# jlogan03/interpn

Hardware: AMD Instinct MI355X
Metric: Mpoints/sec (f64) per GPU + achieved HBM GB/s vs roofline, 3D linear-regular (higher is better)
Workload: dtype f64

## Files before the change

interpn_amd/csrc/abi_layout.hip:

```cpp
#include "abi_internal.h"

using namespace interpn;
using namespace interpn_abi;

namespace interpn_abi {

static bool grid_is_l1_resident(const GridDesc& g) {
  return g.nvals * (g.dtype == kF64 ? 8u : 4u) <= 16u * 1024u;
}

int maybe_build_cubic_tiles(interpn_hip_interp* h) {
  GridDesc& g = h->desc;
  const char* env = getenv("INTERPN_HIP_BRICKS");
  if (env && !strcmp(env, "off")) return INTERPN_HIP_OK;
  if (!(env && strlen(env) == 2) && grid_is_l1_resident(g)) return INTERPN_HIP_OK;
  static const int cand[5][2] = {{4, 4}, {2, 4}, {2, 2}, {1, 4}, {1, 1}};
  size_t free_b = 0, total_b = 0;
  if (hipMemGetInfo(&free_b, &total_b) != hipSuccess) free_b = (size_t)8 << 30;
  int best = -1;
  double best_cost = 0;
  for (int c = 0; c < 5; ++c) {
    const int si = cand[c][0], sj = cand[c][1];
    if (env && strlen(env) == 2 && !(env[0] - '0' == si && env[1] - '0' == sj)) continue;
    unsigned nb[2];
// ... 154 lines not shown
    } else if (fits(bone)) {
      if (bone <= l2_sized || b22 > l2_sized) { si = 1; sj = 1; j4 = f32; }
      else if (b12 <= l2_sized) { si = 1; sj = 2; }
      else { si = 2; sj = 2; }
    } else if (fits(b12)) { si = 1; sj = 2; }
    else if (fits(b22)) { si = 2; sj = 2; }
    else return INTERPN_HIP_OK;
  }
  size_t bytes;
  if (j4) {
    bytes = bj4;
    for (int k = 0; k < 3; ++k) g.brick_nb[k] = nbj4[k];
    g.brick_nb[3] = 0;
    si = sj = 1;
  } else if (cell) {
    bytes = bcell;
    for (int k = 0; k < 4; ++k) g.brick_nb[k] = nbc[k];
    si = sj = 1;
  } else {
    brick_geometry(g, si, sj, g.brick_nb, &bytes);
    g.brick_nb[3] = 0;
  }
  if (bytes / esz >= 0xFFFFFFFFull) return INTERPN_HIP_OK;
  if (bytes > free_b / 2) return INTERPN_HIP_OK;
  g.brick_step[0] = si;
  g.brick_step[1] = sj;
  g.brick_cell = j4 ? 2 : (cell ? 1 : 0);
  hipError_t e = pool_alloc(h->device, &h->bricks_owned, bytes);
  if (e != hipSuccess) { (void)hipGetLastError(); h->bricks_owned = nullptr; g.brick_cell = 0; return INTERPN_HIP_OK; }
  HIP_TRY(build_bricks(g, h->bricks_owned, nullptr));
  HIP_TRY(hipStreamSynchronize(nullptr));
  g.bricks = h->bricks_owned;
  g.sweep_bricks = nullptr;
  int wi = 0, wj = 0, wcell = 0;
  if (!(env && !strcmp(env, "off")) && sweep_layout(g, &wi, &wj, &wcell)) {
    unsigned nbs[3];
    size_t bsw = 0;
    if (wcell == 2) brick_j4_geometry(g, nbs, &bsw);
    else brick_geometry(g, wi, wj, nbs, &bsw);
    if (g.brick_cell == wcell && g.brick_step[0] == wi && g.brick_step[1] == wj) {
      g.sweep_bricks = g.bricks;
    } else if (bsw / esz < 0xFFFFFFFFull && bsw <= free_b / 4 && pool_alloc(h->device, &h->sweep_owned, bsw) == hipSuccess) {
      GridDesc t = g;
      t.brick_cell = wcell;
      t.brick_step[0] = wi;
      t.brick_step[1] = wj;
      for (int k = 0; k < 3; ++k) t.brick_nb[k] = nbs[k];
      t.brick_nb[3] = 0;
      if (build_bricks(t, h->sweep_owned, nullptr) == hipSuccess && hipStreamSynchronize(nullptr) == hipSuccess) {
        g.sweep_bricks = h->sweep_owned;
      } else {
        (void)hipGetLastError();
        pool_free(h->device, h->sweep_owned);
        h->sweep_owned = nullptr;
      }
    } else {
      (void)hipGetLastError();
      h->sweep_owned = nullptr;
    }
    if (g.sweep_bricks) {
      g.sweep_step[0] = wi;
      g.sweep_step[1] = wj;
      g.sweep_cell = wcell;
      for (int k = 0; k < 3; ++k) g.sweep_nb[k] = nbs[k];
      g.sweep_table_bytes = bsw;
    }
  }
  return INTERPN_HIP_OK;
}

}
```

interpn_amd/csrc/abi_options.hip:

```cpp
#include "abi_internal.h"

using namespace interpn;
using namespace interpn_abi;

namespace interpn_abi {

bool option_access(LaunchConfig& c, const char* name, long long* value, bool set) {
  struct Opt { const char* name; int* field; long long lo, hi; };
  const Opt opts[] = {
      {"blocks_per_cu", &c.blocks_per_cu, 1, 65536},
      {"iters_per_block", &c.iters_per_block, 0, 65536},
      {"ppl", &c.ppl, 0, 2},
      {"axis_regs", &c.axis_regs, -1, 2},
      {"force_generic", &c.force_generic, 0, 1},
      {"generic_runtime", &c.generic_runtime, 0, 1},
      {"generic_vec", &c.generic_vec, -1, 1},
      {"persistent", &c.persistent, 0, 1},
      {"axis_lds_kb", &c.axis_lds_kb, -1, 60},
      {"binned", &c.binned, -1, 1},
      {"deal", &c.deal, 0, 1},
      {"bin_slice_log2", &c.bin_slice_log2, 16, 27},
      {"column", &c.column, -1, 1},
      {"column_part", &c.column_part, 0, 1 << 20},
      {"column_threads", &c.column_threads, 256, 1024},
// ... 150 lines not shown
    for (const auto& sl : hm->bin_slots) {
      const unsigned char* base = static_cast<const unsigned char*>(sl.scratch);
      if (!sl.busy && word && base && word >= base && word + sizeof(unsigned) <= base + sl.bytes) idle = true;
    }
    *value = -1;
    if (idle) {
      DeviceGuard guard(h->device);
      if (!guard.ok()) return INTERPN_HIP_ERR_NO_DEVICE;
      unsigned w = 0;
      if (hipDeviceSynchronize() != hipSuccess || hipMemcpy(&w, word, sizeof(w), hipMemcpyDeviceToHost) != hipSuccess) { (void)hipGetLastError(); return INTERPN_HIP_ERR_INVALID_ARGUMENT; }
      *value = w ? 1 : 0;
    }
    return INTERPN_HIP_OK;
  }
  if (!strcmp(name, "sweep_probe_streak")) {
    interpn_hip_interp* hm = const_cast<interpn_hip_interp*>(h);
    std::lock_guard<std::mutex> lk(hm->bin_mu);
    *value = hm->sampling.streak;
    return INTERPN_HIP_OK;
  }
  if (!strcmp(name, "sweep_cell")) { *value = h->desc.sweep_bricks ? h->desc.sweep_cell : 0; return INTERPN_HIP_OK; }
  if (!strcmp(name, "dev_pci")) {
    int dom = 0, bus = 0, dv = 0;
    if (hipDeviceGetAttribute(&dom, hipDeviceAttributePciDomainID, h->device) != hipSuccess ||
        hipDeviceGetAttribute(&bus, hipDeviceAttributePciBusId, h->device) != hipSuccess ||
        hipDeviceGetAttribute(&dv, hipDeviceAttributePciDeviceId, h->device) != hipSuccess) {
      (void)hipGetLastError();
      *value = -1;
    } else {
      *value = ((long long)dom << 16) | ((long long)(bus & 0xFF) << 8) | (long long)(dv & 0xFF);
    }
    return INTERPN_HIP_OK;
  }
  if (!strcmp(name, "sweep_layout")) { *value = h->desc.sweep_bricks ? h->desc.sweep_step[0] * 10 + h->desc.sweep_step[1] : 0; return INTERPN_HIP_OK; }
  if (!strcmp(name, "scratch_allocs")) { *value = h->scratch_allocs.load(); return INTERPN_HIP_OK; }
  if (!strcmp(name, "scratch_bytes")) {
    interpn_hip_interp* hm = const_cast<interpn_hip_interp*>(h);
    std::lock_guard<std::mutex> lk(hm->bin_mu);
    long long tot = 0;
    for (const auto& sl : hm->bin_slots) tot += (long long)sl.bytes;
    *value = tot;
    return INTERPN_HIP_OK;
  }
  LaunchConfig c = h->desc.cfg;
  return option_access(c, name, value, false) ? INTERPN_HIP_OK : INTERPN_HIP_ERR_INVALID_ARGUMENT;
}

int interpn_hip_kernel_name(const interpn_hip_interp* h, char* buf, size_t buflen) {
  if (!h || !buf || buflen == 0) return INTERPN_HIP_ERR_INVALID_ARGUMENT;
  const KernelTag t = h->desc.tag;
  if (!t.name) {
    buf[0] = 0;
    return INTERPN_HIP_OK;
  }
  std::string out = std::string("interpn::") + t.name + "<" + (h->desc.dtype == kF64 ? "double" : "float");
  for (int k = 0; k < t.nargs; ++k) {
    out += ", ";
    if (t.bool_mask & (1u << k)) out += t.args[k] ? "true" : "false";
    else out += std::to_string(t.args[k]);
  }
  out += ">";
  snprintf(buf, buflen, "%s", out.c_str());
  return INTERPN_HIP_OK;
}

size_t interpn_hip_table_bytes(const interpn_hip_interp* h, int* step_i, int* step_j) {
// ... 23 lines not shown
```

interpn_amd/csrc/interpn_device.h:

```cpp
#pragma once

#include <hip/hip_runtime.h>
#include <stdint.h>

#include "cubic_cell_record.h"

namespace interpn {

constexpr int kMaxDims = 8;
constexpr unsigned long long kNoBadIndex = ~0ull;

enum Sat : int { kSatNone = 0, kSatLow = 1, kSatHigh = 2 };

__device__ __forceinline__ void wave_sync() {
  __builtin_amdgcn_fence(__ATOMIC_ACQ_REL, "wavefront");
  __builtin_amdgcn_wave_barrier();
  __builtin_amdgcn_fence(__ATOMIC_ACQ_REL, "wavefront");
}

template <typename V>
__device__ __forceinline__ V stream_load(const V* p) { return __builtin_nontemporal_load(p); }
template <typename V>
__device__ __forceinline__ void stream_store(V* p, V v) { __builtin_nontemporal_store(v, p); }

// ... 40 lines not shown
__device__ __forceinline__ Leaf<T, W> load_leaf(const T* __restrict__ p) {
  typedef typename LeafVec<T, W>::type V;
  V x = *reinterpret_cast<const V*>(p);
  Leaf<T, W> r;
#pragma unroll
  for (int i = 0; i < W; ++i) r.v[i] = x[i];
  return r;
}

template <typename T>
__device__ __forceinline__ bool regular_floc(T x, T start, T step, T* floc_out) {
  T floc = dev_floor<T>((x - start) / step);
  *floc_out = floc;
  return (floc >= (T)-9223372036854775808.0) && (floc < (T)9223372036854775808.0);
}

template <typename T>
__device__ __forceinline__ int clamp_loc(T floc_shifted, int dimmax) {
  const T big = sizeof(T) == 8 ? (T)2147483647.0 : (T)2147483520.0;
  T c = floc_shifted;
  c = c > (T)0 ? c : (T)0;
  c = c < big ? c : big;
  int li = (int)c;
  return li < dimmax ? li : dimmax;
}

template <typename T>
struct StepCell {
  T t;
  int loc;
  bool exact;
};

__device__ __forceinline__ bool exponent_within_256(double a) {
  const unsigned e = ((unsigned)__double2hiint(a) >> 20) & 0x7FFu;
  return e - (1023u - 256u) < 512u;
}

template <bool FMA>
__device__ __forceinline__ StepCell<double> step_cell_fast(double x, double start, double step, double rstep, int dimmax) {
  StepCell<double> r;
  const double qt = (x - start) * rstep;
  const double d = __builtin_amdgcn_fract(qt);
  r.exact = (__builtin_fabs(d - 0.5) < 0.5 - 0x1p-20) && (__builtin_fabs(qt) < 0x1p31);
  int li = (int)qt;
  li = li > 0 ? li : 0;
  li = li < dimmax ? li : dimmax;
  r.loc = li;
  const double lf = (double)li;
  const double izl = mul_add<FMA>(step, lf, start);
  const double a = x - izl;
  r.exact = r.exact && exponent_within_256(a);
  const double q0 = a * rstep;
  const double r0 = __builtin_fma(-step, q0, a);
  const double q1 = __builtin_fma(r0, rstep, q0);
  const double r1 = __builtin_fma(-step, q1, a);
  r.t = __builtin_fma(r1, rstep, q1);
  return r;
}

template <typename T>
struct StepCellIndex {
  T a;
  int loc;
  bool exact;
};
template <bool FMA>
__device__ __forceinline__ StepCellIndex<double> step_cell_index(double x, double start, double step, double rstep, int dimmax) {
  StepCellIndex<double> r;
  const double qt = (x - start) * rstep;
  const double d = __builtin_amdgcn_fract(qt);
  r.exact = (__builtin_fabs(d - 0.5) < 0.5 - 0x1p-20) && (__builtin_fabs(qt) < 0x1p31);
  int li = (int)qt;
  li = li > 0 ? li : 0;
  li = li < dimmax ? li : dimmax;
  r.loc = li;
  const double izl = mul_add<FMA>(step, (double)li, start);
  r.a = x - izl;
  r.exact = r.exact && exponent_within_256(r.a);
  return r;
}
__device__ __forceinline__ double step_cell_quotient(double a, double step, double rstep) {
  const double q0 = a * rstep;
  const double r0 = __builtin_fma(-step, q0, a);
  const double q1 = __builtin_fma(r0, rstep, q0);
  const double r1 = __builtin_fma(-step, q1, a);
  return __builtin_fma(r1, rstep, q1);
}

__device__ __forceinline__ bool exponent_within_24(float a) {
  const unsigned e = (__float_as_uint(a) >> 23) & 0xFFu;
  return e - (127u - 24u) < 48u;
}

template <bool FMA>
__device__ __forceinline__ StepCell<float> step_cell_fast(float x, float start, float step, float rstep, int dimmax) {
  StepCell<float> r;
  const float qt = (x - start) * rstep;
  const float d = __builtin_amdgcn_fractf(qt);
  const float margin = __builtin_fmaf(__builtin_fabsf(qt), 0x1p-21f, 0x1p-21f);
  r.exact = __builtin_fabsf(d - 0.5f) + margin < 0.5f;
  int li = (int)qt;
  li = li > 0 ? li : 0;
  li = li < dimmax ? li : dimmax;
  r.loc = li;
  const float lf = (float)li;
  const float izl = mul_add<FMA>(step, lf, start);
  const float a = x - izl;
  r.exact = r.exact && exponent_within_24(a);
  const float q0 = a * rstep;
  const float r0 = __builtin_fmaf(-step, q0, a);
  const float q1 = __builtin_fmaf(r0, rstep, q0);
  const float r1 = __builtin_fmaf(-step, q1, a);
  r.t = __builtin_fmaf(r1, rstep, q1);
  return r;
}

template <bool FMA>
__device__ __forceinline__ StepCellIndex<float> step_cell_index(float x, float start, float step, float rstep, int dimmax) {
  StepCellIndex<float> r;
  const float qt = (x - start) * rstep;
  const float d = __builtin_amdgcn_fractf(qt);
  const float margin = __builtin_fmaf(__builtin_fabsf(qt), 0x1p-21f, 0x1p-21f);
  r.exact = __builtin_fabsf(d - 0.5f) + margin < 0.5f;
  int li = (int)qt;
  li = li > 0 ? li : 0;
  li = li < dimmax ? li : dimmax;
  r.loc = li;
  const float izl = mul_add<FMA>(step, (float)li, start);
  r.a = x - izl;
  r.exact = r.exact && exponent_within_24(r.a);
  return r;
}
__device__ __forceinline__ float step_cell_quotient(float a, float step, float rstep) {
  const float q0 = a * rstep;
  const float r0 = __builtin_fmaf(-step, q0, a);
  const float q1 = __builtin_fmaf(r0, rstep, q0);
  const float r1 = __builtin_fmaf(-step, q1, a);
  return __builtin_fmaf(r1, rstep, q1);
}

__device__ __forceinline__ bool floor_quotient_fast(double a0, double rb, double* floc) {
  const double qt = a0 * rb;
  const double d = __builtin_amdgcn_fract(qt);
  *floc = __builtin_floor(qt);
  return (__builtin_fabs(d - 0.5) < 0.5 - 0x1p-20) && (__builtin_fabs(qt) < 0x1p31);
}
__device__ __forceinline__ bool floor_quotient_fast(float a0, float rb, float* floc) {
  const float qt = a0 * rb;
  const float d = __builtin_amdgcn_fractf(qt);
  *floc = __builtin_floorf(qt);
  return __builtin_fabsf(d - 0.5f) + __builtin_fmaf(__builtin_fabsf(qt), 0x1p-21f, 0x1p-21f) < 0.5f;
}
__device__ __forceinline__ bool divide_fast(double a, double b, double rb, double* q) {
  const double q0 = a * rb;
  const double r0 = __builtin_fma(-b, q0, a);
  const double q1 = __builtin_fma(r0, rb, q0);
  const double r1 = __builtin_fma(-b, q1, a);
  *q = __builtin_fma(r1, rb, q1);
  return exponent_within_256(a);
}
__device__ __forceinline__ bool divide_fast(float a, float b, float rb, float* q) {
  const float q0 = a * rb;
  const float r0 = __builtin_fmaf(-b, q0, a);
  const float q1 = __builtin_fmaf(r0, rb, q0);
  const float r1 = __builtin_fmaf(-b, q1, a);
// ... 449 lines not shown
```

interpn_amd/csrc/interpn_host.h:

```cpp
#pragma once

#include <hip/hip_runtime.h>
#include <stddef.h>

#include <initializer_list>

namespace interpn {

enum Method : int { kLinear = 0, kCubic = 1, kNearest = 2 };
enum OneDimMethod : int { kLinear1D = 16, kLinearHoldLast1D = 17, kLeft1D = 18, kRight1D = 19, kNearest1D = 20 };
inline bool is_one_dim(int method) { return method >= kLinear1D && method <= kNearest1D; }
enum Kind : int { kRegular = 0, kRectilinear = 1 };
enum DType : int { kF64 = 0, kF32 = 1 };

struct LaunchConfig {
  int num_cus = 256;
  int num_xcds = 8;
  long long l2_bytes = 4ll << 20;
  long long lds_per_cu = 160ll << 10;
  long long lds_per_wg = 64ll << 10;
  int blocks_per_cu = 8;
  int iters_per_block = 0;
  int ppl = 0;
  int axis_regs = -1;
// ... 61 lines not shown
  int n[8] = {0};
  double start[8] = {0};
  double step[8] = {0};
  const void* vals = nullptr;
  size_t nvals = 0;
  const void* grid[8] = {nullptr};
  size_t grid_total = 0;
  const void* axis_image = nullptr;
  unsigned axis_image_bytes = 0;
  unsigned axis_alloc_bytes = 0;
  unsigned axis_g_off[8] = {0};
  unsigned axis_tab_off[8] = {0};
  int axis_buckets[8] = {0};
  double axis_g0[8] = {0};
  double axis_scale[8] = {0};
  unsigned axis_ltab_off[8] = {0};
  double axis_lscale[8] = {0};
  int axis_lscan[8] = {0};
  unsigned axis_rec_off[8] = {0};
  unsigned axis_rec_base = 0;
  unsigned axis_rec_bytes = 0;
  int axis_rec_compact = 0;
  unsigned axis_recg_off[8] = {0};
  unsigned axis_crec_off[8] = {0};
  unsigned axis_crec_bytes = 0;
  const void* bricks = nullptr;
  int rec1_buckets = 0;
  double rec1_scale = 0.0;
  int brick_step[2] = {2, 2};
  unsigned brick_nb[4] = {0, 0, 0, 0};
  const void* bricks11 = nullptr;
  unsigned bricks11_nb[2] = {0, 0};
  int brick_cell = 0;
  const void* sweep_bricks = nullptr;
  int sweep_step[2] = {0, 0};
  int sweep_cell = 0;
  unsigned sweep_nb[3] = {0, 0, 0};
  size_t sweep_table_bytes = 0;
  double bound_lo[8] = {0};
  double bound_hi[8] = {0};
  int unrep_status = 7;
  double od_start = 0, od_step = 0, od_stop = 0, od_rstep = 0;
  int od_fast = 0;
  int od_M = 0;
  double od_g0 = 0, od_scale = 0;
  size_t od_g_off = 0, od_tab_off = 0, od_table_bytes = 0;
  LaunchConfig cfg;
  mutable KernelTag tag;
  mutable int last_lattice_path = -1;
  mutable int last_points_path = -1;
  mutable int last_binned = 0;
};

inline unsigned brick_iters(const GridDesc& g, size_t npts, int points_per_lane, int setup) {
  unsigned iters = g.cfg.iters_per_block > 0 ? (unsigned)g.cfg.iters_per_block : (setup == 2 ? 8u : (setup == 1 ? 4u : 1u));
  const size_t rows = (npts + (size_t)256 * points_per_lane - 1) / ((size_t)256 * points_per_lane);
  while ((rows + iters - 1) / iters > (1u << 23)) iters *= 2;
  return iters;
}

constexpr unsigned long long kNoBadIndexHost = ~0ull;

constexpr size_t kMaxGridLdsBytes = 20 * 1024;
constexpr size_t kMaxGridLdsBytesWide = 60 * 1024;

struct Thresholds {
  size_t table_l2_sized;
  size_t table_l2_share;
  double table_l2_model;
  size_t binned_table_min;
  size_t binned_points_min;
// ... 188 lines not shown
```

interpn_amd/csrc/k_linear_brick.hip:

```cpp
#include <cstdlib>

#include "linear_brick.h"

namespace interpn {

static unsigned bricks_along(int n, int step) {
  if (step == 1) return (unsigned)(n - 1);
  if (step == 2) return (unsigned)((n - 1) / 2 + 1);
  return (unsigned)((n - 2) / step + 1);
}

void brick_geometry(const GridDesc& g, int si, int sj, unsigned nb[3], size_t* bytes) {
  const int N = g.ndims;
  const int kw = g.dtype == kF64 ? 4 : 8;
  nb[0] = bricks_along(g.n[N - 3], si);
  nb[1] = bricks_along(g.n[N - 2], sj);
  nb[2] = bricks_along(g.n[N - 1], kw - 1);
  size_t lead = 1;
  for (int d = 0; d < N - 3; ++d) lead *= (size_t)g.n[d];
  *bytes = lead * nb[0] * nb[1] * nb[2] * 128;
}

void brick_cell_geometry(const GridDesc& g, unsigned nb[4], size_t* bytes) {
  const int N = g.ndims;
// ... 6 lines not shown
  for (int d = 0; d < N - 4; ++d) lead *= (size_t)g.n[d];
  *bytes = lead * nb[3] * nb[0] * nb[1] * nb[2] * 128;
}

void brick_j4_geometry(const GridDesc& g, unsigned nb[3], size_t* bytes) {
  const int N = g.ndims;
  nb[0] = bricks_along(g.n[N - 3], 1);
  nb[1] = bricks_along(g.n[N - 2], 3);
  nb[2] = bricks_along(g.n[N - 1], 3);
  size_t lead = 1;
  for (int d = 0; d < N - 3; ++d) lead *= (size_t)g.n[d];
  *bytes = lead * nb[0] * nb[1] * nb[2] * 128;
}

static hipError_t build_cell_bricks(const GridDesc& g, void* bricks, hipStream_t stream) {
  const int N = g.ndims;
  size_t lead = 1;
  for (int d = 0; d < N - 4; ++d) lead *= (size_t)g.n[d];
  const size_t elems = lead * g.brick_nb[3] * g.brick_nb[0] * g.brick_nb[1] * g.brick_nb[2] * (g.dtype == kF64 ? 16 : 32);
  size_t blocks = (elems + kBlock - 1) / kBlock;
  if (blocks > 65535) blocks = 65535;
  if (g.dtype == kF64)
    hipLaunchKernelGGL(k_build_cell_bricks<double>, dim3((unsigned)blocks), dim3(kBlock), 0, stream,
                       static_cast<const double*>(g.vals), static_cast<double*>(bricks), lead, g.n[N - 4], g.n[N - 3],
                       g.n[N - 2], g.n[N - 1], g.brick_nb[3], g.brick_nb[0], g.brick_nb[1], g.brick_nb[2]);
  else
    hipLaunchKernelGGL(k_build_cell_bricks<float>, dim3((unsigned)blocks), dim3(kBlock), 0, stream,
                       static_cast<const float*>(g.vals), static_cast<float*>(bricks), lead, g.n[N - 4], g.n[N - 3],
                       g.n[N - 2], g.n[N - 1], g.brick_nb[3], g.brick_nb[0], g.brick_nb[1], g.brick_nb[2]);
  return hipGetLastError();
}

hipError_t build_bricks(const GridDesc& g, void* bricks, hipStream_t stream) {
  if (g.brick_cell == 1) return build_cell_bricks(g, bricks, stream);
  const int N = g.ndims;
  if (g.brick_cell == 2) {
    if (g.dtype != kF32) return hipErrorInvalidValue;
    size_t lead4 = 1;
    for (int d = 0; d < N - 3; ++d) lead4 *= (size_t)g.n[d];
    const size_t elems4 = lead4 * g.brick_nb[0] * g.brick_nb[1] * g.brick_nb[2] * 32;
    size_t blocks4 = (elems4 + kBlock - 1) / kBlock;
    if (blocks4 > 65535) blocks4 = 65535;
    hipLaunchKernelGGL(k_build_j4_bricks<float>, dim3((unsigned)blocks4), dim3(kBlock), 0, stream,
                       static_cast<const float*>(g.vals), static_cast<float*>(bricks), lead4, g.n[N - 3], g.n[N - 2],
                       g.n[N - 1], g.brick_nb[0], g.brick_nb[1], g.brick_nb[2]);
    return hipGetLastError();
  }
  size_t lead = 1;
  for (int d = 0; d < N - 3; ++d) lead *= (size_t)g.n[d];
  const size_t elems = lead * g.brick_nb[0] * g.brick_nb[1] * g.brick_nb[2] * (g.dtype == kF64 ? 16 : 32);
  size_t blocks = (elems + kBlock - 1) / kBlock;
  if (blocks > 65535) blocks = 65535;
  if (g.dtype == kF64)
    hipLaunchKernelGGL(k_build_bricks<double>, dim3((unsigned)blocks), dim3(kBlock), 0, stream,
                       static_cast<const double*>(g.vals), static_cast<double*>(bricks), lead, g.n[N - 3], g.n[N - 2],
                       g.n[N - 1], g.brick_step[0], g.brick_step[1], g.brick_nb[0], g.brick_nb[1], g.brick_nb[2]);
  else
    hipLaunchKernelGGL(k_build_bricks<float>, dim3((unsigned)blocks), dim3(kBlock), 0, stream,
                       static_cast<const float*>(g.vals), static_cast<float*>(bricks), lead, g.n[N - 3], g.n[N - 2],
                       g.n[N - 1], g.brick_step[0], g.brick_step[1], g.brick_nb[0], g.brick_nb[1], g.brick_nb[2]);
  return hipGetLastError();
}

template <typename T, int N, bool RECT, bool FMA, int PPL, int AXR>
static hipError_t launch_steps(const GridDesc& g, const BrickArgs<T, N>& a, size_t lds, unsigned blocks, hipStream_t stream) {
  const int si = g.brick_step[0], sj = g.brick_step[1];
  if constexpr (sizeof(T) == 4) {
    if (g.brick_cell == 2) {
      g.tag.set("k_linear_brick", {N, RECT, FMA, 1, 1, PPL, AXR, 0, 2}, 0b000000110u);
      hipLaunchKernelGGL((k_linear_brick<T, N, RECT, FMA, 1, 1, PPL, AXR, 0, 2>), dim3(blocks), dim3(kBlock), lds, stream, a);
      return hipGetLastError();
    }
  }
  if constexpr (N >= 4) {
    if (g.brick_cell == 1) {
      g.tag.set("k_linear_brick", {N, RECT, FMA, 1, 1, PPL, AXR, 0, 1}, 0b000000110u);
      hipLaunchKernelGGL((k_linear_brick<T, N, RECT, FMA, 1, 1, PPL, AXR, 0, 1>), dim3(blocks), dim3(kBlock), lds, stream, a);
      return hipGetLastError();
    }
  }
  g.tag.set("k_linear_brick", {N, RECT, FMA, si == 1 ? 1 : 2, (si == 1 && sj == 1) ? 1 : 2, PPL, AXR, 0, 0}, 0b000000110u);
  if (si == 1 && sj == 1) hipLaunchKernelGGL((k_linear_brick<T, N, RECT, FMA, 1, 1, PPL, AXR>), dim3(blocks), dim3(kBlock), lds, stream, a);
  else if (si == 1 && sj == 2) hipLaunchKernelGGL((k_linear_brick<T, N, RECT, FMA, 1, 2, PPL, AXR>), dim3(blocks), dim3(kBlock), lds, stream, a);
  else hipLaunchKernelGGL((k_linear_brick<T, N, RECT, FMA, 2, 2, PPL, AXR>), dim3(blocks), dim3(kBlock), lds, stream, a);
  return hipGetLastError();
}

template <typename T, int N, int PPL>
static hipError_t launch_kind(const GridDesc& g, BrickArgs<T, N>& a, size_t lds, size_t axis_lds, size_t npts, hipStream_t stream) {
  const int axr = lane_axes_mode(g);
  a.iters = brick_iters(g, npts, PPL, g.kind != kRectilinear ? 0 : (axr == 0 ? 2 : 1));
  if ((a.gate || g.launch_fat) && g.cfg.gated_iters > 0 && a.iters < (unsigned)g.cfg.gated_iters) a.iters = (unsigned)g.cfg.gated_iters;
  const size_t nslots = (npts + PPL - 1) / PPL;
// ... 76 lines not shown
```

interpn_amd/csrc/k_linear_sweep.hip:

```cpp
#include <cstdlib>
#include <cstring>

#include "linear_sweep.h"

namespace interpn {

namespace {

constexpr int kSweepRows = 12;
constexpr int kSweepParked = 4;
#ifndef INTERPN_SWEEP_RECT_PARKED
#define INTERPN_SWEEP_RECT_PARKED 2
#endif
#ifndef INTERPN_SWEEP_RECT_ROWS
#define INTERPN_SWEEP_RECT_ROWS 12
#endif
constexpr int kSweepParkedRect = INTERPN_SWEEP_RECT_PARKED;
#ifndef INTERPN_SWEEP_F32_ROWS
#define INTERPN_SWEEP_F32_ROWS 24
#endif
#ifndef INTERPN_SWEEP_F32_PARKED
#define INTERPN_SWEEP_F32_PARKED 0
#endif
constexpr int kSweepRowsF32 = INTERPN_SWEEP_F32_ROWS;
// ... 31 lines not shown
  if (const char* env = getenv("INTERPN_HIP_SWEEP_LAYOUT")) {
    if (!strcmp(env, "11") || !strcmp(env, "12")) { *si = 1; *sj = env[1] - '0'; return true; }
  }
  const size_t window = kSweepPointsPerCu * (size_t)(g.cfg.num_cus > 0 ? g.cfg.num_cus : 256) * 85 / 100;
  const size_t l11 = brick_lines(g, 1, 1), l12 = brick_lines(g, 1, 2);
  const int xcds = g.cfg.num_xcds > 0 ? g.cfg.num_xcds : 8;
  if ((size_t)xcds * l11 * 2 <= window) { *si = 1; *sj = 1; }
  else if ((size_t)xcds * l12 * 10 <= window * 7) { *si = 1; *sj = 2; }
  else { *si = 1; *sj = 1; }
  return true;
}

int linear3_sweep_applies(const GridDesc& g, size_t npts) {
  if (!g.sweep_bricks || g.cfg.sweep == 0 || g.cfg.force_generic) return 0;
  if (g.sweep_table_bytes >= (1ull << 32)) return 0;
  for (int d = 0; d < 3; ++d)
    if (g.n[d] >= (1 << 20)) return 0;
  if ((unsigned long long)g.sweep_nb[0] * g.sweep_nb[1] >= (1ull << 24) || g.sweep_nb[2] >= (1u << 24)) return 0;
  const size_t lds = g.kind == kRectilinear
                         ? (lane_axes_mode(g) != 0
                                ? (size_t)SweepLds<double, INTERPN_SWEEP_LANES_ROWS, INTERPN_SWEEP_LANES_PARKED>::kWave * (kSweepThreads / 64) + SweepLds<double, INTERPN_SWEEP_LANES_ROWS, INTERPN_SWEEP_LANES_PARKED>::kWorkgroup
                                : (size_t)SweepLds<double, INTERPN_SWEEP_RECT_ROWS, kSweepParkedRect>::kWave * (kSweepThreads / 64) + SweepLds<double, INTERPN_SWEEP_RECT_ROWS, kSweepParkedRect>::kWorkgroup + kSweepAxisLds)
                         : (size_t)SweepLds<double, kSweepRows, kSweepParked>::kWave * (kSweepThreads / 64) + SweepLds<double, kSweepRows, kSweepParked>::kWorkgroup;
  if ((long long)lds > g.cfg.lds_per_cu) return 0;
  if (g.cfg.sweep > 0) return 2;
  const bool beyond_l2 = g.sweep_table_bytes > thresholds(g.cfg).table_l2_sized;
  const size_t cus = (size_t)(g.cfg.num_cus > 0 ? g.cfg.num_cus : 256);
  const size_t per_cu = g.dtype == kF64 ? (size_t)(g.kind == kRectilinear ? INTERPN_SWEEP_RECT_ROWS + kSweepParkedRect : kSweepRows + kSweepParked) * kSweepThreads : kSweepPointsPerCuF32;
  const size_t rounds = g.dtype == kF64 ? (beyond_l2 ? 4 : 8) : (beyond_l2 ? 3 : 6);
  if (npts < rounds * per_cu * cus) return 1;
  return 2;
}

template <typename T, bool RECT, bool FMA, int SI, int SJ, int AXR, int CELL = 0>
static hipError_t go(const GridDesc& g, const SweepArgs<T>& s, unsigned blocks, hipStream_t stream) {
  constexpr int K = sweep_rows<T, RECT, AXR>(), KL = sweep_parked<T, RECT, AXR>(), TH = kSweepThreads;
  auto kern = k_linear_sweep<T, RECT, FMA, SI, SJ, K, TH, AXR, false, CELL, KL>;
  const size_t lds = (size_t)SweepLds<T, K, KL>::kWave * (TH / 64) + SweepLds<T, K, KL>::kWorkgroup + ((RECT && AXR == 4 && s.b.ax.use_lds) ? (size_t)s.b.ax.image_bytes : 0);
  const size_t most = (size_t)SweepLds<T, K, KL>::kWave * (TH / 64) + SweepLds<T, K, KL>::kWorkgroup + (RECT && AXR == 4 ? kSweepAxisLds : 0);
  hipError_t e = allow_dynamic_lds(reinterpret_cast<const void*>(kern), most);
  if (e != hipSuccess) return e;
  g.tag.set("k_linear_sweep", {RECT, FMA, SI, SJ, K, TH, AXR, 0, CELL, KL, 0}, 0b00010000011u);
  hipLaunchKernelGGL(kern, dim3(blocks), dim3(TH), lds, stream, s);
  return hipGetLastError();
}

template <typename T, bool RECT, bool FMA, int AXR>
static hipError_t go_layout(const GridDesc& g, const SweepArgs<T>& s, unsigned blocks, hipStream_t stream) {
  if constexpr (sizeof(T) == 4) {
    if (g.sweep_cell == 2) return go<T, RECT, FMA, 1, 1, AXR, 2>(g, s, blocks, stream);
    return hipErrorInvalidValue;
  } else {
    if (g.sweep_cell != 0) return hipErrorInvalidValue;
    if (g.sweep_step[0] == 1 && g.sweep_step[1] == 1) return go<T, RECT, FMA, 1, 1, AXR>(g, s, blocks, stream);
    if (g.sweep_step[0] == 1 && g.sweep_step[1] == 2) return go<T, RECT, FMA, 1, 2, AXR>(g, s, blocks, stream);
    return hipErrorInvalidValue;
  }
}

constexpr unsigned kProbeRows = 256;
template <typename T, int N>
struct ProbeArgs {
  const T* obs[N];
  size_t npts;
  T start[N], scale[N];
  int top[N];
  int sk;
  SweepWork* work;
  unsigned* host_word;
  unsigned seq;
};

template <typename T, int N>
__global__ void __launch_bounds__(256) k_sweep_probe(const ProbeArgs<T, N> p) {
  const unsigned lane = threadIdx.x & 63u;
  const unsigned row = blockIdx.x * 4u + (threadIdx.x >> 6);
  const unsigned rows = gridDim.x * 4u;
  const size_t slots = p.npts / 64u;
  const size_t at = (size_t)((unsigned long long)row * (slots - 1u) / (rows > 1u ? rows - 1u : 1u)) * 64u + lane;
  unsigned id = 0;
#pragma unroll
  for (int d = 0; d < N; ++d) {
    const T u = (p.obs[d][at] - p.start[d]) * p.scale[d];
    const int c = u >= (T)1 ? (u < (T)p.top[d] ? (int)u : p.top[d]) : 0;
    id = id * 0x9E3779B1u + (unsigned)(d == N - 1 ? c / p.sk : c);
  }
// ... 109 lines not shown
```

interpn_amd/csrc/linear_brick.h:

```cpp
#pragma once

#include "lane_axes.h"
#include "rect_args.h"

namespace interpn {

template <typename T, int CELL = 0> struct BrickGeom {
  static constexpr int KW = CELL == 2 ? 4 : (CELL ? 16 : 32) / (int)sizeof(T);
  static constexpr int SK = KW - 1;
  static constexpr int IJ = 4 * KW;
  static constexpr int ELEMS = CELL == 2 ? 32 : (CELL ? 2 : 1) * IJ;
};

template <typename T, int N>
struct BrickArgs {
  const T* bricks;
  const T* obs[N];
  T* out;
  unsigned long long* first_bad;
  size_t npts;
  T start[N];
  T step[N];
  int n[N];
  AxisArgs<T, N> ax;
// ... 294 lines not shown
      }
      T r[2];
#pragma unroll
      for (int dk = 0; dk < 2; ++dk) {
        const T c0 = mul_add<FMA>(t[N - 3], c.v[1][0][dk] - c.v[0][0][dk], c.v[0][0][dk]);
        const T c1 = mul_add<FMA>(t[N - 3], c.v[1][1][dk] - c.v[0][1][dk], c.v[0][1][dk]);
        r[dk] = mul_add<FMA>(t[N - 2], c1 - c0, c0);
      }
      resv[h] = mul_add<FMA>(t[N - 1], r[1] - r[0], r[0]);
    }
    if constexpr (ABL == 2) {
      if (resv[0] == (T)1234567.25 && resv[PPL - 1] == (T)-7654321.5) a.out[i0] = resv[0];
    } else if (PPL >= 2) {
      typedef T TV __attribute__((ext_vector_type(PPL)));
      if (live[PPL - 1]) {
        TV v;
#pragma unroll
        for (int h = 0; h < PPL; ++h) v[h] = resv[h];
        stream_store(reinterpret_cast<TV*>(a.out + i0), v);
      } else {
#pragma unroll
        for (int h = 0; h < PPL; ++h)
          if (live[h]) stream_store(a.out + i0 + h, resv[h]);
      }
    } else if (live[0]) {
      stream_store(a.out + i0, resv[0]);
    }
  }
}

template <typename T>
__global__ void __launch_bounds__(kBlock) k_build_bricks(const T* __restrict__ vals, T* __restrict__ bricks, size_t nlead,
                                                         int n0, int n1, int n2, int si, int sj, unsigned nbi, unsigned nbj,
                                                         unsigned nbk) {
  constexpr int KW = BrickGeom<T>::KW;
  constexpr int EL = BrickGeom<T>::ELEMS;
  const size_t per_lead = (size_t)nbi * nbj * nbk * EL;
  const size_t total = nlead * per_lead;
  for (size_t e = (size_t)blockIdx.x * kBlock + threadIdx.x; e < total; e += (size_t)gridDim.x * kBlock) {
    const size_t lead = e / per_lead;
    size_t b = e - lead * per_lead;
    const unsigned within = (unsigned)(b % EL);
    b /= EL;
    const unsigned bk = (unsigned)(b % nbk); b /= nbk;
    const unsigned bj = (unsigned)(b % nbj); b /= nbj;
    const unsigned bi = (unsigned)b;
    const int i = (int)bi * si + (int)(within / (2 * KW));
    const int j = (int)bj * sj + (int)((within / KW) & 1);
    const int k = (int)bk * (KW - 1) + (int)(within % KW);
    T v = (T)0;
    if (i < n0 && j < n1 && k < n2) v = vals[((lead * n0 + i) * n1 + j) * n2 + k];
    bricks[e] = v;
  }
}

template <typename T>
__global__ void __launch_bounds__(kBlock) k_build_j4_bricks(const T* __restrict__ vals, T* __restrict__ bricks, size_t nlead,
                                                            int n0, int n1, int n2, unsigned nbi, unsigned nbj, unsigned nbk) {
  const size_t per_lead = (size_t)nbi * nbj * nbk * 32;
  const size_t total = nlead * per_lead;
  for (size_t e = (size_t)blockIdx.x * kBlock + threadIdx.x; e < total; e += (size_t)gridDim.x * kBlock) {
    const size_t lead = e / per_lead;
    size_t b = e - lead * per_lead;
    const unsigned within = (unsigned)(b & 31);
    b >>= 5;
    const unsigned bk = (unsigned)(b % nbk); b /= nbk;
    const unsigned bj = (unsigned)(b % nbj); b /= nbj;
    const unsigned bi = (unsigned)b;
    const int i = (int)bi + (int)(within >> 4);
    const int j = (int)bj * 3 + (int)((within >> 2) & 3);
    const int k = (int)bk * 3 + (int)(within & 3);
    T v = (T)0;
    if (i < n0 && j < n1 && k < n2) v = vals[((lead * n0 + i) * n1 + j) * n2 + k];
    bricks[e] = v;
  }
}

template <typename T>
__global__ void __launch_bounds__(kBlock) k_build_cell_bricks(const T* __restrict__ vals, T* __restrict__ bricks, size_t nlead,
                                                              int nh, int n0, int n1, int n2, unsigned nbh, unsigned nbi,
                                                              unsigned nbj, unsigned nbk) {
  typedef BrickGeom<T, 1> G;
  const size_t per_lead = (size_t)nbh * nbi * nbj * nbk * G::ELEMS;
  const size_t total = nlead * per_lead;
// ... 22 lines not shown
```

interpn_amd/csrc/linear_sweep.h:

```cpp
#pragma once

#include "linear_brick.h"
#include "sweep_rounds.h"

namespace interpn {


template <typename T>
struct SweepArgs {
  BrickArgs<T, 3> b;
  T key_start, key_scale;
  int key_shift;
  T rstep[3];
  unsigned fastdiv;
  unsigned rounds;
  unsigned per_shard;
  unsigned period;
  unsigned period_default;
  unsigned gated;
  SweepWork* work;
  unsigned long long* stamps;
};

template <typename T, int K, int KL = 0>
struct SweepLds {
  static constexpr unsigned kRowOnly = 64u * K * sizeof(T);
  static constexpr unsigned kPiece = 64u * kPieceRow * 2u * sizeof(T);
  static constexpr unsigned kRow = kRowOnly > kPiece ? kRowOnly : kPiece;
  static constexpr unsigned kPark = 64u * KL * 3u * sizeof(T);
  static constexpr unsigned kOff = 64u * 16u;
  static constexpr unsigned kWave = kRow + kPark + kOff;
  static constexpr unsigned kWorkgroup = 16;
  static_assert(kRow + kPark >= 64u * (K + KL) * sizeof(T), "the result exchange spans the row buffer and the parked rows' bytes");
  static_assert(64u * 4u * 2u <= kOff, "the sort's counters live in the piece offsets' bytes");
  static_assert(64u * (K + KL) * 2u <= kRow, "the 16-bit source-index exchange of a round stays inside the row buffer (the parked coordinates sit right behind it)");
};

template <typename T, bool RECT, bool FMA, int SI, int SJ, int K, int THREADS, int AXR = 0, bool STAMPS = false, int CELL = 0, int KL = 0, int ABL = 0>
__global__ void __launch_bounds__(THREADS) k_linear_sweep(const SweepArgs<T> s) {
  constexpr int PPV = 16 / (int)sizeof(T);
  constexpr int KT = K + KL;
  static_assert(KT % PPV == 0 && KT % 2 == 0 && K >= PPV && KT <= 32 && KL >= 0, "rows per wave and round");
  static_assert(CELL == 0 || (CELL == 2 && sizeof(T) == 4 && SI == 1 && SJ == 1), "2 x 4 x 4 bricks: f32");
  static_assert(RECT == (AXR != 0), "rectilinear grids: lane-resident axes only");
  typedef typename LeafVec<T, 2>::type P;
  typedef T TV __attribute__((ext_vector_type(PPV)));
  typedef BrickGeom<T, CELL> Geom;
  constexpr int SK = Geom::SK;
  typedef SweepLds<T, K, KL> L;
  const BrickArgs<T, 3>& a = s.b;
  if (s.gated && __hip_atomic_load(&s.work->take_brick, __ATOMIC_RELAXED, __HIP_MEMORY_SCOPE_AGENT) != 0u) return;
  extern __shared__ __attribute__((aligned(16))) unsigned char smem_raw[];
  const unsigned lane = threadIdx.x & 63u;
  const unsigned wave = threadIdx.x >> 6;
  unsigned char* const mine = smem_raw + wave * L::kWave;
  T* const row = reinterpret_cast<T*>(mine);
  typedef unsigned short __attribute__((may_alias)) lds_u16;
  lds_u16* const row16 = reinterpret_cast<lds_u16*>(mine);
  P* const lds_piece = reinterpret_cast<P*>(mine);
  T* const park = reinterpret_cast<T*>(mine + L::kRow);
  lds_u32* const lds_off = reinterpret_cast<lds_u32*>(mine + L::kRow + L::kPark);
  lds_u32* const cnt = lds_off;
  lds_u32* const wg_words = reinterpret_cast<lds_u32*>(smem_raw + (THREADS / 64) * L::kWave);
  if (threadIdx.x < 4) wg_words[threadIdx.x] = 0;
  if constexpr (RECT && AXR == 4) {
    if (s.b.ax.use_lds) {
      const unsigned words = s.b.ax.image_bytes >> 2;
      const unsigned* src = reinterpret_cast<const unsigned*>(s.b.ax.image);
      unsigned* dst = reinterpret_cast<unsigned*>(smem_raw + (THREADS / 64) * L::kWave + L::kWorkgroup);
      for (unsigned k = threadIdx.x; k < words; k += THREADS) dst[k] = src[k];
    }
  }
  __syncthreads();
  const unsigned q = lane & 3u;
  const unsigned quad = lane >> 2;
  constexpr size_t kChunk = (size_t)64 * KT;
  const unsigned nwaves = gridDim.x * (THREADS / 64);
// ... 150 lines not shown
      constexpr bool RECT_T_LATE = RECT && (sizeof(T) == 4 || AXR == 4 || INTERPN_SWEEP_LANES_LATE);
      T t[3];
      int loc[3];
      T av[3] = {(T)0, (T)0, (T)0};
      T bv[3] = {(T)1, (T)1, (T)1};
      bool have_t = false;
      if constexpr (RECT && AXR == 4) {
#pragma unroll
        for (int d = 0; d < 3; ++d) {
          const Axis<T> ax = make_axis<T, 3>(a.ax, axis_base, d);
          T x0, x1;
          loc[d] = axis_cell<T>(ax, xr[d], &x0, &x1);
          av[d] = xr[d] - x0;
          bv[d] = x1 - x0;
        }
      } else if constexpr (RECT) {
        T xin[1][3], x0_r[1][3], x1_r[1][3];
        int cell_r[1][3];
#pragma unroll
        for (int d = 0; d < 3; ++d) xin[0][d] = xr[d];
        lane_axes_locate<T, 3, 1, AXR>(a.ax, la, xin, cell_r, x0_r, x1_r);
#pragma unroll
        for (int d = 0; d < 3; ++d) {
          av[d] = xr[d] - x0_r[0][d];
          bv[d] = x1_r[0][d] - x0_r[0][d];
          if constexpr (!RECT_T_LATE) t[d] = av[d] / bv[d];
          loc[d] = cell_r[0][d];
        }
      } else {
        bool ok = true;
        bool exact = false;
        if constexpr (ABL != 3) {
          exact = s.fastdiv != 0;
#pragma unroll
          for (int d = 0; d < 3; ++d) {
            const StepCellIndex<T> sc = step_cell_index<FMA>(xr[d], a.start[d], a.step[d], s.rstep[d], a.n[d] - 2);
            av[d] = sc.a;
            loc[d] = sc.loc;
            exact = exact && sc.exact;
          }
        }
        if (__any(!exact)) {
          have_t = true;
#pragma unroll
          for (int d = 0; d < 3; ++d) {
            T floc;
            if constexpr (ABL == 3) {
              const T rs = (T)1 / a.step[d];
              floc = dev_floor<T>((xr[d] - a.start[d]) * rs);
              const int l = clamp_loc<T>(floc, a.n[d] - 2);
              const T izl = mul_add<FMA>(a.step[d], (T)l, a.start[d]);
              t[d] = (xr[d] - izl) * rs;
              loc[d] = l;
              continue;
            }
            ok &= regular_floc<T>(xr[d], a.start[d], a.step[d], &floc);
            const int l = clamp_loc<T>(floc, a.n[d] - 2);
            const T izl = mul_add<FMA>(a.step[d], (T)l, a.start[d]);
            t[d] = (xr[d] - izl) / a.step[d];
            loc[d] = l;
          }
        }
        const size_t gi = base + ((src[k / 2] >> (16 * (k & 1))) & 0xFFFFu);
        if (!ok && gi < a.npts) atomicMin(a.first_bad, (unsigned long long)gi);
      }
      const unsigned bk = (unsigned)loc[2] / (unsigned)SK;
      Cell<T> c;
      if constexpr (SI == 1 && SJ == 1 && ABL != 1) {
        const unsigned mine_b = brick_line_bytes24<T, CELL>(a.nbj, a.nbk, loc[0], loc[1], loc[2]);
        const unsigned char* const tb = reinterpret_cast<const unsigned char*>(a.bricks);
        const unsigned mypiece = (CELL == 2 ? ((q >> 1) * 4u + (q & 1u)) * 4u : q * (unsigned)Geom::KW) * (unsigned)sizeof(T);
        P pc[4];
        pc[0] = *reinterpret_cast<const P*>(tb + ((unsigned)__builtin_amdgcn_mov_dpp((int)mine_b, 0x00, 0xF, 0xF, true) + mypiece));
        pc[1] = *reinterpret_cast<const P*>(tb + ((unsigned)__builtin_amdgcn_mov_dpp((int)mine_b, 0x55, 0xF, 0xF, true) + mypiece));
        pc[2] = *reinterpret_cast<const P*>(tb + ((unsigned)__builtin_amdgcn_mov_dpp((int)mine_b, 0xAA, 0xF, 0xF, true) + mypiece));
        pc[3] = *reinterpret_cast<const P*>(tb + ((unsigned)__builtin_amdgcn_mov_dpp((int)mine_b, 0xFF, 0xF, 0xF, true) + mypiece));
        if constexpr (RECT && RECT_T_LATE) {
          __builtin_amdgcn_sched_barrier(0);
#pragma unroll
          for (int d = 0; d < 3; ++d) t[d] = av[d] / bv[d];
          __builtin_amdgcn_sched_barrier(0);
        }
        if constexpr (!RECT && ABL != 3) {
          __builtin_amdgcn_sched_barrier(0);
          if (!have_t) {
#pragma unroll
            for (int d = 0; d < 3; ++d) t[d] = step_cell_quotient(av[d], a.step[d], s.rstep[d]);
          }
          __builtin_amdgcn_sched_barrier(0);
        }
#pragma unroll
        for (int r = 0; r < 4; ++r) lds_piece[(quad * 4 + r) * kPieceRow + q] = pc[r];
        wave_sync();
#pragma unroll
        for (int p = 0; p < 4; ++p) {
          const P w = lds_piece[(quad * 4 + q) * kPieceRow + p];
          c.v[p >> 1][p & 1][0] = w.x;
          c.v[p >> 1][p & 1][1] = w.y;
        }
        wave_sync();
      } else {
        if constexpr (RECT && RECT_T_LATE) {
#pragma unroll
          for (int d = 0; d < 3; ++d) t[d] = av[d] / bv[d];
        }
        if constexpr (!RECT && ABL != 3) {
          if (!have_t) {
#pragma unroll
            for (int d = 0; d < 3; ++d) t[d] = step_cell_quotient(av[d], a.step[d], s.rstep[d]);
          }
        }
        const unsigned kpart = bk * (unsigned)Geom::ELEMS + ((unsigned)loc[2] - bk * (unsigned)SK);
#pragma unroll
        for (int p = 0; p < 4; ++p)
          lds_off[(quad * 4 + p) * 4 + q] = brick_piece<T, SI, SJ, CELL>(a.nbj, a.nbk, loc[0], loc[1], kpart, p >> 1, p & 1);
        wave_sync();
        const uint4 toff = *reinterpret_cast<const uint4*>(&lds_off[(quad * 4 + q) * 4]);
        if constexpr (ABL == 1) {
#pragma unroll
          for (int e = 0; e < 8; ++e) c.v[e >> 2][(e >> 1) & 1][e & 1] = t[e % 3] + (T)(toff.x & 7u) + (T)e;
        } else {
          c = gather_cell<T>(a.bricks, toff, 0u, lds_piece, quad, q);
        }
      }
      T rr2[2];
#pragma unroll
      for (int dk = 0; dk < 2; ++dk) {
        const T c0 = mul_add<FMA>(t[0], c.v[1][0][dk] - c.v[0][0][dk], c.v[0][0][dk]);
        const T c1 = mul_add<FMA>(t[0], c.v[1][1][dk] - c.v[0][1][dk], c.v[0][1][dk]);
        rr2[dk] = mul_add<FMA>(t[1], c1 - c0, c0);
      }
      res[k] = mul_add<FMA>(t[2], rr2[1] - rr2[0], rr2[0]);
      asm volatile("" : "+v"(res[k]));
    }
    if constexpr (STAMPS) { const unsigned long long now = __builtin_amdgcn_s_memrealtime(); st_rows += now - st_mark; st_mark = now; }
    __builtin_amdgcn_s_setprio(2);
#pragma unroll
    for (int k = 0; k < KT; ++k) row[(src[k / 2] >> (16 * (k & 1))) & 0xFFFFu] = res[k];
    wave_sync();
#pragma unroll
    for (int kv = 0; kv < KT / PPV; ++kv) {
      const size_t i0 = base + (size_t)kv * (64 * PPV) + PPV * lane;
      const TV v = *reinterpret_cast<const TV*>(&row[kv * (64 * PPV) + PPV * lane]);
      if constexpr (ABL == 2) {
        if (v[0] == (T)123.456) stream_store(reinterpret_cast<TV*>(a.out + i0), v);
      } else if (full || i0 + PPV - 1 < a.npts) {
        stream_store(reinterpret_cast<TV*>(a.out + i0), v);
      } else {
#pragma unroll
        for (int h = 0; h < PPV; ++h)
          if (i0 + h < a.npts) stream_store(a.out + i0 + h, v[h]);
      }
    }
    wave_sync();
  }
  const unsigned long long t_end = __builtin_amdgcn_s_memrealtime();
  if (lane == 0) {
    const unsigned my_ticks = (unsigned)(t_end - t_begin);
    atomicAdd(&wg_words[0], my_ticks);
    atomicAdd(&wg_words[1], my_rounds);
    __builtin_amdgcn_fence(__ATOMIC_RELEASE, "workgroup");
    if (atomicAdd(&wg_words[2], 1u) == THREADS / 64 - 1) {
// ... 34 lines not shown
```

Before: 109,800.

## Store plane differences in sweep brick table and merge exactness guards

Result: no change. 110,200 (median of 6 runs) (+0.3%).

```diff
diff --git a/interpn_amd/csrc/abi_layout.hip b/interpn_amd/csrc/abi_layout.hip
--- a/interpn_amd/csrc/abi_layout.hip
+++ b/interpn_amd/csrc/abi_layout.hip
@@ -210,7 +210,8 @@
   HIP_TRY(hipStreamSynchronize(nullptr));
   g.bricks = h->bricks_owned;
   g.sweep_bricks = nullptr;
-  int wi = 0, wj = 0, wcell = 0;
+  g.sweep_diff = 0;
+  int wi = 0, wj = 0, wcell = 0, sweep_diff = 0;
   if (!(env && !strcmp(env, "off")) && sweep_layout(g, &wi, &wj, &wcell)) {
     unsigned nbs[3];
     size_t bsw = 0;
@@ -225,6 +226,9 @@
       t.brick_step[1] = wj;
       for (int k = 0; k < 3; ++k) t.brick_nb[k] = nbs[k];
       t.brick_nb[3] = 0;
+      const char* env_diff = getenv("INTERPN_HIP_SWEEP_DIFF");
+      t.brick_diff = (wcell == 0 && wi == 1 && wj == 1 && !(env_diff && !strcmp(env_diff, "off"))) ? 1 : 0;
+      sweep_diff = t.brick_diff;
       if (build_bricks(t, h->sweep_owned, nullptr) == hipSuccess && hipStreamSynchronize(nullptr) == hipSuccess) {
         g.sweep_bricks = h->sweep_owned;
       } else {
@@ -242,6 +246,7 @@
       g.sweep_cell = wcell;
       for (int k = 0; k < 3; ++k) g.sweep_nb[k] = nbs[k];
       g.sweep_table_bytes = bsw;
+      g.sweep_diff = g.sweep_bricks == g.bricks ? 0 : sweep_diff;
     }
   }
   return INTERPN_HIP_OK;
diff --git a/interpn_amd/csrc/abi_options.hip b/interpn_amd/csrc/abi_options.hip
--- a/interpn_amd/csrc/abi_options.hip
+++ b/interpn_amd/csrc/abi_options.hip
@@ -206,6 +206,7 @@
     }
     return INTERPN_HIP_OK;
   }
+  if (!strcmp(name, "sweep_diff")) { *value = h->desc.sweep_bricks ? h->desc.sweep_diff : 0; return INTERPN_HIP_OK; }
   if (!strcmp(name, "sweep_layout")) { *value = h->desc.sweep_bricks ? h->desc.sweep_step[0] * 10 + h->desc.sweep_step[1] : 0; return INTERPN_HIP_OK; }
   if (!strcmp(name, "scratch_allocs")) { *value = h->scratch_allocs.load(); return INTERPN_HIP_OK; }
   if (!strcmp(name, "scratch_bytes")) {
diff --git a/interpn_amd/csrc/interpn_device.h b/interpn_amd/csrc/interpn_device.h
--- a/interpn_amd/csrc/interpn_device.h
+++ b/interpn_amd/csrc/interpn_device.h
@@ -96,8 +96,18 @@
   bool exact;
 };
 
-__device__ __forceinline__ bool exponent_within_256(double a) {
-  const unsigned e = ((unsigned)__double2hiint(a) >> 20) & 0x7FFu;
+__host__ __device__ __forceinline__ unsigned exponent_field(double a) {
+  unsigned long long b;
+  __builtin_memcpy(&b, &a, sizeof(b));
+  return ((unsigned)(b >> 32) >> 20) & 0x7FFu;
+}
+__host__ __device__ __forceinline__ unsigned exponent_field(float a) {
+  unsigned b;
+  __builtin_memcpy(&b, &a, sizeof(b));
+  return (b >> 23) & 0xFFu;
+}
+__host__ __device__ __forceinline__ bool exponent_within_256(double a) {
+  const unsigned e = exponent_field(a);
   return e - (1023u - 256u) < 512u;
 }
 
@@ -130,7 +140,7 @@
   bool exact;
 };
 template <bool FMA>
-__device__ __forceinline__ StepCellIndex<double> step_cell_index(double x, double start, double step, double rstep, int dimmax) {
+__device__ __forceinline__ StepCellIndex<double> step_cell_index_unguarded(double x, double start, double step, double rstep, int dimmax) {
   StepCellIndex<double> r;
   const double qt = (x - start) * rstep;
   const double d = __builtin_amdgcn_fract(qt);
@@ -141,8 +151,19 @@
   r.loc = li;
   const double izl = mul_add<FMA>(step, (double)li, start);
   r.a = x - izl;
+  return r;
+}
+template <bool FMA>
+__device__ __forceinline__ StepCellIndex<double> step_cell_index(double x, double start, double step, double rstep, int dimmax) {
+  StepCellIndex<double> r = step_cell_index_unguarded<FMA>(x, start, step, rstep, dimmax);
   r.exact = r.exact && exponent_within_256(r.a);
   return r;
+}
+__host__ __device__ __forceinline__ unsigned min3u(unsigned a, unsigned b, unsigned c) { const unsigned m = a < b ? a : b; return m < c ? m : c; }
+__host__ __device__ __forceinline__ unsigned max3u(unsigned a, unsigned b, unsigned c) { const unsigned m = a > b ? a : b; return m > c ? m : c; }
+__host__ __device__ __forceinline__ bool exponents_within_256(double a0, double a1, double a2) {
+  const unsigned e0 = exponent_field(a0), e1 = exponent_field(a1), e2 = exponent_field(a2);
+  return min3u(e0, e1, e2) >= 1023u - 256u && max3u(e0, e1, e2) < 1023u + 256u;
 }
 __device__ __forceinline__ double step_cell_quotient(double a, double step, double rstep) {
   const double q0 = a * rstep;
@@ -152,8 +173,8 @@
   return __builtin_fma(r1, rstep, q1);
 }
 
-__device__ __forceinline__ bool exponent_within_24(float a) {
-  const unsigned e = (__float_as_uint(a) >> 23) & 0xFFu;
+__host__ __device__ __forceinline__ bool exponent_within_24(float a) {
+  const unsigned e = exponent_field(a);
   return e - (127u - 24u) < 48u;
 }
 
@@ -181,7 +202,7 @@
 }
 
 template <bool FMA>
-__device__ __forceinline__ StepCellIndex<float> step_cell_index(float x, float start, float step, float rstep, int dimmax) {
+__device__ __forceinline__ StepCellIndex<float> step_cell_index_unguarded(float x, float start, float step, float rstep, int dimmax) {
   StepCellIndex<float> r;
   const float qt = (x - start) * rstep;
   const float d = __builtin_amdgcn_fractf(qt);
@@ -193,9 +214,20 @@
   r.loc = li;
   const float izl = mul_add<FMA>(step, (float)li, start);
   r.a = x - izl;
+  return r;
+}
+template <bool FMA>
+__device__ __forceinline__ StepCellIndex<float> step_cell_index(float x, float start, float step, float rstep, int dimmax) {
+  StepCellIndex<float> r = step_cell_index_unguarded<FMA>(x, start, step, rstep, dimmax);
   r.exact = r.exact && exponent_within_24(r.a);
   return r;
 }
+__host__ __device__ __forceinline__ bool exponents_within_24(float a0, float a1, float a2) {
+  const unsigned e0 = exponent_field(a0), e1 = exponent_field(a1), e2 = exponent_field(a2);
+  return min3u(e0, e1, e2) >= 127u - 24u && max3u(e0, e1, e2) < 127u + 24u;
+}
+__host__ __device__ __forceinline__ bool dividends_in_range(double a0, double a1, double a2) { return exponents_within_256(a0, a1, a2); }
+__host__ __device__ __forceinline__ bool dividends_in_range(float a0, float a1, float a2) { return exponents_within_24(a0, a1, a2); }
 __device__ __forceinline__ float step_cell_quotient(float a, float step, float rstep) {
   const float q0 = a * rstep;
   const float r0 = __builtin_fmaf(-step, q0, a);
diff --git a/interpn_amd/csrc/interpn_host.h b/interpn_amd/csrc/interpn_host.h
--- a/interpn_amd/csrc/interpn_host.h
+++ b/interpn_amd/csrc/interpn_host.h
@@ -117,11 +117,13 @@
   const void* bricks11 = nullptr;
   unsigned bricks11_nb[2] = {0, 0};
   int brick_cell = 0;
+  int brick_diff = 0;
   const void* sweep_bricks = nullptr;
   int sweep_step[2] = {0, 0};
   int sweep_cell = 0;
   unsigned sweep_nb[3] = {0, 0, 0};
   size_t sweep_table_bytes = 0;
+  int sweep_diff = 0;
   double bound_lo[8] = {0};
   double bound_hi[8] = {0};
   int unrep_status = 7;
diff --git a/interpn_amd/csrc/k_linear_brick.hip b/interpn_amd/csrc/k_linear_brick.hip
--- a/interpn_amd/csrc/k_linear_brick.hip
+++ b/interpn_amd/csrc/k_linear_brick.hip
@@ -62,6 +62,7 @@
 }
 
 hipError_t build_bricks(const GridDesc& g, void* bricks, hipStream_t stream) {
+  if (g.brick_diff && g.brick_cell != 0) return hipErrorInvalidValue;
   if (g.brick_cell == 1) return build_cell_bricks(g, bricks, stream);
   const int N = g.ndims;
   if (g.brick_cell == 2) {
@@ -76,6 +77,8 @@
                        g.n[N - 1], g.brick_nb[0], g.brick_nb[1], g.brick_nb[2]);
     return hipGetLastError();
   }
+  const int diff = g.brick_diff ? 1 : 0;
+  if (diff && g.brick_step[0] != 1) return hipErrorInvalidValue;
   size_t lead = 1;
   for (int d = 0; d < N - 3; ++d) lead *= (size_t)g.n[d];
   const size_t elems = lead * g.brick_nb[0] * g.brick_nb[1] * g.brick_nb[2] * (g.dtype == kF64 ? 16 : 32);
@@ -84,11 +87,11 @@
   if (g.dtype == kF64)
     hipLaunchKernelGGL(k_build_bricks<double>, dim3((unsigned)blocks), dim3(kBlock), 0, stream,
                        static_cast<const double*>(g.vals), static_cast<double*>(bricks), lead, g.n[N - 3], g.n[N - 2],
-                       g.n[N - 1], g.brick_step[0], g.brick_step[1], g.brick_nb[0], g.brick_nb[1], g.brick_nb[2]);
+                       g.n[N - 1], g.brick_step[0], g.brick_step[1], g.brick_nb[0], g.brick_nb[1], g.brick_nb[2], diff);
   else
     hipLaunchKernelGGL(k_build_bricks<float>, dim3((unsigned)blocks), dim3(kBlock), 0, stream,
                        static_cast<const float*>(g.vals), static_cast<float*>(bricks), lead, g.n[N - 3], g.n[N - 2],
-                       g.n[N - 1], g.brick_step[0], g.brick_step[1], g.brick_nb[0], g.brick_nb[1], g.brick_nb[2]);
+                       g.n[N - 1], g.brick_step[0], g.brick_step[1], g.brick_nb[0], g.brick_nb[1], g.brick_nb[2], diff);
   return hipGetLastError();
 }
 
diff --git a/interpn_amd/csrc/k_linear_sweep.hip b/interpn_amd/csrc/k_linear_sweep.hip
--- a/interpn_amd/csrc/k_linear_sweep.hip
+++ b/interpn_amd/csrc/k_linear_sweep.hip
@@ -87,15 +87,15 @@
   return 2;
 }
 
-template <typename T, bool RECT, bool FMA, int SI, int SJ, int AXR, int CELL = 0>
+template <typename T, bool RECT, bool FMA, int SI, int SJ, int AXR, int CELL = 0, bool DIFF = false>
 static hipError_t go(const GridDesc& g, const SweepArgs<T>& s, unsigned blocks, hipStream_t stream) {
   constexpr int K = sweep_rows<T, RECT, AXR>(), KL = sweep_parked<T, RECT, AXR>(), TH = kSweepThreads;
-  auto kern = k_linear_sweep<T, RECT, FMA, SI, SJ, K, TH, AXR, false, CELL, KL>;
+  auto kern = k_linear_sweep<T, RECT, FMA, SI, SJ, K, TH, AXR, false, CELL, KL, 0, DIFF>;
   const size_t lds = (size_t)SweepLds<T, K, KL>::kWave * (TH / 64) + SweepLds<T, K, KL>::kWorkgroup + ((RECT && AXR == 4 && s.b.ax.use_lds) ? (size_t)s.b.ax.image_bytes : 0);
   const size_t most = (size_t)SweepLds<T, K, KL>::kWave * (TH / 64) + SweepLds<T, K, KL>::kWorkgroup + (RECT && AXR == 4 ? kSweepAxisLds : 0);
   hipError_t e = allow_dynamic_lds(reinterpret_cast<const void*>(kern), most);
   if (e != hipSuccess) return e;
-  g.tag.set("k_linear_sweep", {RECT, FMA, SI, SJ, K, TH, AXR, 0, CELL, KL, 0}, 0b00010000011u);
+  g.tag.set("k_linear_sweep", {RECT, FMA, SI, SJ, K, TH, AXR, 0, CELL, KL, 0, DIFF}, 0b100010000011u);
   hipLaunchKernelGGL(kern, dim3(blocks), dim3(TH), lds, stream, s);
   return hipGetLastError();
 }
@@ -107,6 +107,10 @@
     return hipErrorInvalidValue;
   } else {
     if (g.sweep_cell != 0) return hipErrorInvalidValue;
+    if (g.sweep_diff) {
+      if (g.sweep_step[0] == 1 && g.sweep_step[1] == 1) return go<T, RECT, FMA, 1, 1, AXR, 0, true>(g, s, blocks, stream);
+      return hipErrorInvalidValue;
+    }
     if (g.sweep_step[0] == 1 && g.sweep_step[1] == 1) return go<T, RECT, FMA, 1, 1, AXR>(g, s, blocks, stream);
     if (g.sweep_step[0] == 1 && g.sweep_step[1] == 2) return go<T, RECT, FMA, 1, 2, AXR>(g, s, blocks, stream);
     return hipErrorInvalidValue;
diff --git a/interpn_amd/csrc/linear_brick.h b/interpn_amd/csrc/linear_brick.h
--- a/interpn_amd/csrc/linear_brick.h
+++ b/interpn_amd/csrc/linear_brick.h
@@ -350,7 +350,7 @@
 template <typename T>
 __global__ void __launch_bounds__(kBlock) k_build_bricks(const T* __restrict__ vals, T* __restrict__ bricks, size_t nlead,
                                                          int n0, int n1, int n2, int si, int sj, unsigned nbi, unsigned nbj,
-                                                         unsigned nbk) {
+                                                         unsigned nbk, int diff) {
   constexpr int KW = BrickGeom<T>::KW;
   constexpr int EL = BrickGeom<T>::ELEMS;
   const size_t per_lead = (size_t)nbi * nbj * nbk * EL;
@@ -368,6 +368,11 @@
     const int k = (int)bk * (KW - 1) + (int)(within % KW);
     T v = (T)0;
     if (i < n0 && j < n1 && k < n2) v = vals[((lead * n0 + i) * n1 + j) * n2 + k];
+    if (diff && within >= 2 * KW) {
+      T below = (T)0;
+      if (i - 1 < n0 && j < n1 && k < n2) below = vals[((lead * n0 + (i - 1)) * n1 + j) * n2 + k];
+      v = v - below;
+    }
     bricks[e] = v;
   }
 }
diff --git a/interpn_amd/csrc/linear_sweep.h b/interpn_amd/csrc/linear_sweep.h
--- a/interpn_amd/csrc/linear_sweep.h
+++ b/interpn_amd/csrc/linear_sweep.h
@@ -36,13 +36,14 @@
   static_assert(64u * (K + KL) * 2u <= kRow, "the 16-bit source-index exchange of a round stays inside the row buffer (the parked coordinates sit right behind it)");
 };
 
-template <typename T, bool RECT, bool FMA, int SI, int SJ, int K, int THREADS, int AXR = 0, bool STAMPS = false, int CELL = 0, int KL = 0, int ABL = 0>
+template <typename T, bool RECT, bool FMA, int SI, int SJ, int K, int THREADS, int AXR = 0, bool STAMPS = false, int CELL = 0, int KL = 0, int ABL = 0, bool DIFF = false>
 __global__ void __launch_bounds__(THREADS) k_linear_sweep(const SweepArgs<T> s) {
   constexpr int PPV = 16 / (int)sizeof(T);
   constexpr int KT = K + KL;
   static_assert(KT % PPV == 0 && KT % 2 == 0 && K >= PPV && KT <= 32 && KL >= 0, "rows per wave and round");
   static_assert(CELL == 0 || (CELL == 2 && sizeof(T) == 4 && SI == 1 && SJ == 1), "2 x 4 x 4 bricks: f32");
   static_assert(RECT == (AXR != 0), "rectilinear grids: lane-resident axes only");
+  static_assert(!DIFF || (SI == 1 && SJ == 1 && CELL == 0 && ABL != 1), "plane differences: the one-line-per-cell 2 x 2 x KW table");
   typedef typename LeafVec<T, 2>::type P;
   typedef T TV __attribute__((ext_vector_type(PPV)));
   typedef BrickGeom<T, CELL> Geom;
@@ -259,13 +260,18 @@
         bool exact = false;
         if constexpr (ABL != 3) {
           exact = s.fastdiv != 0;
+#ifndef INTERPN_SWEEP_ONE_GUARD
+#define INTERPN_SWEEP_ONE_GUARD 1
+#endif
 #pragma unroll
           for (int d = 0; d < 3; ++d) {
-            const StepCellIndex<T> sc = step_cell_index<FMA>(xr[d], a.start[d], a.step[d], s.rstep[d], a.n[d] - 2);
+            const StepCellIndex<T> sc = INTERPN_SWEEP_ONE_GUARD ? step_cell_index_unguarded<FMA>(xr[d], a.start[d], a.step[d], s.rstep[d], a.n[d] - 2)
+                                                                : step_cell_index<FMA>(xr[d], a.start[d], a.step[d], s.rstep[d], a.n[d] - 2);
             av[d] = sc.a;
             loc[d] = sc.loc;
             exact = exact && sc.exact;
           }
+          if (INTERPN_SWEEP_ONE_GUARD) exact = exact && dividends_in_range(av[0], av[1], av[2]);
         }
         if (__any(!exact)) {
           have_t = true;
@@ -287,9 +293,11 @@
             t[d] = (xr[d] - izl) / a.step[d];
             loc[d] = l;
           }
-        }
-        const size_t gi = base + ((src[k / 2] >> (16 * (k & 1))) & 0xFFFFu);
-        if (!ok && gi < a.npts) atomicMin(a.first_bad, (unsigned long long)gi);
+          if (!ok) {
+            const size_t gi = base + ((src[k / 2] >> (16 * (k & 1))) & 0xFFFFu);
+            if (gi < a.npts) atomicMin(a.first_bad, (unsigned long long)gi);
+          }
+        }
       }
       const unsigned bk = (unsigned)loc[2] / (unsigned)SK;
       Cell<T> c;
@@ -351,10 +359,13 @@
         }
       }
       T rr2[2];
+      if constexpr (DIFF) __builtin_amdgcn_sched_barrier(0);
 #pragma unroll
       for (int dk = 0; dk < 2; ++dk) {
-        const T c0 = mul_add<FMA>(t[0], c.v[1][0][dk] - c.v[0][0][dk], c.v[0][0][dk]);
-        const T c1 = mul_add<FMA>(t[0], c.v[1][1][dk] - c.v[0][1][dk], c.v[0][1][dk]);
+        const T d0 = DIFF ? c.v[1][0][dk] : c.v[1][0][dk] - c.v[0][0][dk];
+        const T d1 = DIFF ? c.v[1][1][dk] : c.v[1][1][dk] - c.v[0][1][dk];
+        const T c0 = mul_add<FMA>(t[0], d0, c.v[0][0][dk]);
+        const T c1 = mul_add<FMA>(t[0], d1, c.v[0][1][dk]);
         rr2[dk] = mul_add<FMA>(t[1], c1 - c0, c0);
       }
       res[k] = mul_add<FMA>(t[2], rr2[1] - rr2[0], rr2[0]);
```
